# Graph-COM/HEPT

Hardware: AMD Instinct MI355X
Metric: attention-fwd points/sec (higher is better)
Workload: dtype bf16

## Files before the change

### hept_amd/csrc/block_attn.hip

```cpp
#include "common.h"
#include "p2p_dev.h"

namespace {

#ifndef HEPT_ATTN_STORE
#define HEPT_ATTN_STORE 1
#endif
__device__ __forceinline__ void store16_rows(unsigned int* dst, const u32x4& v) {
#if HEPT_ATTN_STORE == 1
    __builtin_nontemporal_store(v, reinterpret_cast<u32x4*>(dst));
#else
    *reinterpret_cast<u32x4*>(dst) = v;
#endif
}

#ifndef HEPT_RAGGED16_WAVES
#define HEPT_RAGGED16_WAVES 7
#endif
constexpr int attn_waves(int nkt, bool bf16, bool p16, bool full, bool diff = false) {
    if (diff) return full ? 3 : 2;
    return bf16 ? ((nkt == 3 && !p16 && full) ? 6 : (full ? 8 : HEPT_RAGGED16_WAVES)) : (full ? 6 : 4);
}
template <int NKT, bool BF16, bool P16, bool F16QK, bool FULL, bool DIFF = false>
__global__ __launch_bounds__(64 * NKT) __attribute__((amdgpu_waves_per_eu(attn_waves(NKT, BF16, P16, FULL, DIFF), attn_waves(NKT, BF16, P16, FULL, DIFF))))
void block_attn_kernel(const char* __restrict__ qhat,
                                                              const char* __restrict__ kvhat,
                                                              const int* __restrict__ qpos,
                                                              const int* __restrict__ kpos,
                                                              float* __restrict__ part, int N, int H, int D, int B,
                                                              int nb, HeadRange hr, PushArgs pa) {
    if (pa.push_wgs > 0 && (int)blockIdx.x < pa.push_wgs) {
        reduce_push_body<P16>(pa, (int)blockIdx.x);
        return;
    }
    constexpr int NT = 64 * NKT;
    constexpr int KEYS = 32 * NKT;
    constexpr int ESZ = BF16 ? 2 : 4;
    constexpr int QROW = 32 * ESZ;
    constexpr int KVROW = 2 * QROW;
    constexpr int CH = QROW / 16;
    constexpr int CPR = 2 * CH;

    extern __shared__ __attribute__((aligned(16))) char smem[];
    char* k_s = smem;
    char* v_s = smem + KEYS * QROW;
    float* kn_s = reinterpret_cast<float*>(smem + 2 * KEYS * QROW);
    int* qidx_s = reinterpret_cast<int*>(smem + 2 * KEYS * QROW + KEYS * 4);

    const int tid = threadIdx.x, lane = tid & 63, w = tid >> 6, hh = lane >> 5, li = lane & 31;
    const int bid = (int)blockIdx.x - pa.push_wgs;
    const int h = hr.h0 + bid % hr.hg;
    const int rest = bid / hr.hg;
    const int b = hr.tl > 0 ? rest / hr.tl : rest % nb, t = hr.tl > 0 ? rest % hr.tl : rest / nb;
    const size_t seg = ((size_t)t * H + h) * N + (size_t)b * B;
    const int* __restrict__ kp = kpos + seg;
    const int* __restrict__ qp = qpos + seg;
    const char* __restrict__ qbase = qhat + (size_t)h * N * QROW;
    const char* __restrict__ kvbase = kvhat + (size_t)h * N * KVROW;

    const int qi = w * 32 + li;
    const bool qvalid = FULL || qi < B;
    const int qsrc = qp[qvalid ? qi : 0];
    if (hh == 0) qidx_s[qi] = qvalid ? qsrc : -1;
    const char* qrow = qbase + (size_t)qsrc * QROW;
    float qn = *reinterpret_cast<const float*>(qrow + QROW - 4);
    u32x4 qraw[BF16 ? 2 : 4];
#pragma unroll
    for (int s = 0; s < (BF16 ? 2 : 4); ++s)
        qraw[s] = *reinterpret_cast<const u32x4*>(qrow + (BF16 ? (s * 32 + hh * 16) : (hh * 64 + s * 16)));
    if (hh == 1) qraw[BF16 ? 1 : 3][3] = 0u;
    if constexpr (DIFF) {
        static_assert(!BF16, "the difference form runs on f32 rows");
        float part = 0.f;
#pragma unroll
        for (int s2 = 0; s2 < 4; ++s2)
#pragma unroll
            for (int j = 0; j < 4; ++j) {
                const bool feat = 16 * hh + 4 * s2 + j < D;
                const float qv = __uint_as_float(qraw[s2][j]);
                part = feat ? fmaf(qv, qv, part) : part;
                if (!feat) qraw[s2][j] = 0u;
            }
        qn = -0.5f * (part + __shfl_xor(part, 32));
    }

#pragma unroll
    for (int it = 0; it < CPR / 2; ++it) {
        const int ci = it * NT + tid;
        const int key = ci / CPR, c = ci % CPR;
        u32x4 val = {0u, 0u, 0u, 0u};
        if (FULL || key < B) {
            const int src = kp[key];
            val = *reinterpret_cast<const u32x4*>(kvbase + (size_t)src * KVROW + c * 16);
        }
        if (c < CH) {
            if (c == CH - 1) {
                kn_s[key] = __uint_as_float(val[3]);
                val[3] = 0u;
            }
            const int sw = BF16 ? ((key >> 2) & 3) : ((key >> 1) & 7);
            *reinterpret_cast<u32x4*>(k_s + key * QROW + ((c ^ sw) * 16)) = val;
        } else {
            *reinterpret_cast<u32x4*>(v_s + key * QROW + (c - CH) * 16) = val;
        }
    }
    __syncthreads();
    if constexpr (DIFF) {
        if (tid < KEYS) {
            const int sw = (tid >> 1) & 7;
            float acc = 0.f;
            for (int col = 0; col < D; ++col) {
                const float kv2 = *reinterpret_cast<const float*>(k_s + tid * QROW + (((col >> 2) ^ sw) * 16) + (col & 3) * 4);
                acc = fmaf(kv2, kv2, acc);
            }
            kn_s[tid] = -0.5f * acc;
        }
        __syncthreads();
    }

    f32x16 z;
#pragma unroll
    for (int r = 0; r < 16; ++r) z[r] = 0.f;

#pragma unroll
    for (int kt = 0; kt < NKT; ++kt) {
        if (!FULL && kt * 32 >= B) break;
        const int key = kt * 32 + li;
        f32x16 x;
#pragma unroll
        for (int r = 0; r < 16; ++r) x[r] = qn + kn_s[kt * 32 + hept_acc_row(r, hh)];

        if constexpr (BF16) {
#pragma unroll
            for (int s = 0; s < 2; ++s) {
                const int c = 2 * s + hh;
                const u32x4 kraw =
                    *reinterpret_cast<const u32x4*>(k_s + key * QROW + ((c ^ ((key >> 2) & 3)) * 16));
                if constexpr (F16QK)
                    x = __builtin_amdgcn_mfma_f32_32x32x16_f16(__builtin_bit_cast(f16x8, kraw),
                                                               __builtin_bit_cast(f16x8, qraw[s]), x, 0, 0, 0);
                else
                    x = __builtin_amdgcn_mfma_f32_32x32x16_bf16(__builtin_bit_cast(bf16x8, kraw),
                                                                __builtin_bit_cast(bf16x8, qraw[s]), x, 0, 0, 0);
            }
        } else {
            float kf[16];
#pragma unroll
            for (int c = 0; c < 4; ++c) {
                const f32x4 kk = *reinterpret_cast<const f32x4*>(
                    k_s + key * QROW + (((4 * hh + c) ^ ((key >> 1) & 7)) * 16));
                kf[4 * c] = kk[0]; kf[4 * c + 1] = kk[1]; kf[4 * c + 2] = kk[2]; kf[4 * c + 3] = kk[3];
            }
#pragma unroll
            for (int s = 0; s < 16; ++s)
                x = __builtin_amdgcn_mfma_f32_32x32x2f32(kf[s], __uint_as_float(qraw[s >> 2][s & 3]), x, 0, 0, 0);
            if constexpr (DIFF) {
                float dsq[16];
#pragma unroll
                for (int r = 0; r < 16; ++r) dsq[r] = 0.f;
                for (int col = D; col < 30; ++col) {
                    const float qc = *reinterpret_cast<const float*>(qrow + col * 4);
#pragma unroll
                    for (int r = 0; r < 16; ++r) {
                        const int kr = kt * 32 + hept_acc_row(r, hh);
                        const float kc = *reinterpret_cast<const float*>(
                            k_s + kr * QROW + (((col >> 2) ^ ((kr >> 1) & 7)) * 16) + (col & 3) * 4);
                        const float dlt = qc - kc;
                        dsq[r] = fmaf(dlt, dlt, dsq[r]);
                    }
                }
#pragma unroll
                for (int r = 0; r < 16; ++r) x[r] = fmaf(-0.5f, dsq[r], x[r]);
            }
        }

        float pr[16];
        exp_clamped(x, pr);
        if (!FULL && (kt + 1) * 32 > B) {
#pragma unroll
            for (int r = 0; r < 16; ++r)
                if (kt * 32 + hept_acc_row(r, hh) >= B) pr[r] = 0.f;
        }

        if constexpr (BF16) {
            const int g = lane >> 4, l16 = lane & 15;
            const int vrow = kt * 32 + 4 * hh + (l16 >> 2);
            const int vcol = 32 * (g & 1) + 8 * (l16 & 3);
#pragma unroll
            for (int s = 0; s < 2; ++s) {
                u32x4 pw;
#pragma unroll
                for (int j = 0; j < 4; ++j) pw[j] = hept_pack_bf16(pr[8 * s + 2 * j], pr[8 * s + 2 * j + 1]);
                const s16x4 v0 = __builtin_amdgcn_ds_read_tr16_b64_v4i16(
                    (lds_s16x4_ptr)(v_s + (vrow + 16 * s) * QROW + vcol));
                const s16x4 v1 = __builtin_amdgcn_ds_read_tr16_b64_v4i16(
                    (lds_s16x4_ptr)(v_s + (vrow + 16 * s + 8) * QROW + vcol));
                typedef __attribute__((ext_vector_type(8))) short s16x8;
                const s16x8 vv = {v0[0], v0[1], v0[2], v0[3], v1[0], v1[1], v1[2], v1[3]};
                z = __builtin_amdgcn_mfma_f32_32x32x16_bf16(__builtin_bit_cast(bf16x8, pw),
                                                            __builtin_bit_cast(bf16x8, vv), z, 0, 0, 0);
            }
        } else {
#pragma unroll
            for (int r = 0; r < 16; ++r) {
                const float vv =
                    *reinterpret_cast<const float*>(v_s + (kt * 32 + hept_acc_row(r, hh)) * QROW + li * 4);
                z = __builtin_amdgcn_mfma_f32_32x32x2f32(pr[r], vv, z, 0, 0, 0);
            }
        }
    }

    if constexpr (P16) {
        __syncthreads();
        float* tile = reinterpret_cast<float*>(smem) + w * 32 * 32;
        {
            float* wr = tile + (4 * hh) * 32 + li;
#pragma unroll
            for (int r = 0; r < 16; ++r) wr[((r & 3) + 8 * (r >> 2)) * 32] = z[r];
        }
        unsigned int* __restrict__ pt =
            reinterpret_cast<unsigned int*>(part) + (size_t)t * hr.tstride_rows * 16 + (size_t)(h - hr.hsub) * 16;
#pragma unroll
        for (int j = 0; j < 2; ++j) {
            const int row = (lane >> 2) + 16 * j, pc = lane & 3;
            const int q2 = w * 32 + row;
            const f32x4 f0 = *reinterpret_cast<const f32x4*>(tile + row * 32 + pc * 8);
            const f32x4 f1 = *reinterpret_cast<const f32x4*>(tile + row * 32 + pc * 8 + 4);
            u32x4 v = {hept_pack_bf16(f0[0], f0[1]), hept_pack_bf16(f0[2], f0[3]), hept_pack_bf16(f1[0], f1[1]),
                       hept_pack_bf16(f1[2], f1[3])};
            if (pc == 3) v = u32x4{__float_as_uint(f0[0] + 1e-20f), 0u, 0u, 0u};
            if (FULL || q2 < B) {
                const int dst = qidx_s[q2];
                if (pa.direct) {
                    bool remote;
                    char* rowp = direct_row(pa, dst, h - hr.h0, 64, remote) + pc * 16;
                    if (remote) store16_system(rowp, v);
                    else *reinterpret_cast<u32x4*>(rowp) = v;
                } else {
                    store16_rows(pt + (size_t)dst * hr.hout * 16 + pc * 4, v);
                }
            }
        }
    } else {
        float* __restrict__ pt = part + (size_t)t * hr.tstride_rows * 32 + (size_t)(h - hr.hsub) * 32 + li;
#pragma unroll
        for (int r = 0; r < 16; ++r) {
            const int q2 = w * 32 + hept_acc_row(r, hh);
            if (FULL || q2 < B) {
                const int dst = qidx_s[q2];
                float val = z[r];
                if (li == D) val += 1e-20f;
                if (pa.direct) {
                    bool remote;
                    char* rowp = direct_row(pa, dst, h - hr.h0, 128, remote) + li * 4;
                    if (remote) store4_system(rowp, __float_as_uint(val));
                    else *reinterpret_cast<float*>(rowp) = val;
                } else {
                    pt[(size_t)dst * hr.hout * 32] = val;
                }
            }
        }
    }
    if (pa.direct) {
        drain_remote_stores();
        if (pa.counter) signal_when_all_done(pa.counter, pa.peers, pa.world, pa.flag_idx, pa.epoch, gridDim.x - pa.push_wgs);
    }
}

#ifndef HEPT_SPLIT_CK8
#define HEPT_SPLIT_CK8 128
#endif
constexpr int split_ck(int nkt) { return nkt == 8 ? HEPT_SPLIT_CK8 : (nkt >= 2 ? 64 : 32); }
#ifndef HEPT_SPLIT_PP
#define HEPT_SPLIT_PP 2
#endif
template <int NKT, bool FULL, int VP, bool DIFF = false>
__global__ __launch_bounds__(64 * NKT) void block_attn_split_kernel(const float* __restrict__ qhat,
                                                                    const float* __restrict__ kvhat,
                                                                    const int* __restrict__ qpos,
                                                                    const int* __restrict__ kpos,
                                                                    float* __restrict__ part, int N, int H, int D,
                                                                    int B, int nb, HeadRange hr, PushArgs pa) {
    if (pa.push_wgs > 0 && (int)blockIdx.x < pa.push_wgs) {
        reduce_push_body<false>(pa, (int)blockIdx.x);
        return;
    }
    constexpr int NT = 64 * NKT;
    constexpr int KEYS = 32 * NKT;
    constexpr int PROW = 64;
    constexpr int CK = split_ck(NKT);
    constexpr int NCH = (KEYS + CK - 1) / CK;
    constexpr int IPT = (CK * 8 + NT - 1) / NT;
    extern __shared__ __attribute__((aligned(16))) char smem[];
    char* k_s = smem;
    char* v_s = smem + 3 * CK * PROW;
    float* kc_s = reinterpret_cast<float*>(smem + (3 + VP) * CK * PROW);

    const int tid = threadIdx.x, lane = tid & 63, w = tid >> 6, hh = lane >> 5, li = lane & 31;
    const int bid = (int)blockIdx.x - pa.push_wgs;
    const int h = hr.h0 + bid % hr.hg;
    const int rest = bid / hr.hg;
    const int b = hr.tl > 0 ? rest / hr.tl : rest % nb, t = hr.tl > 0 ? rest % hr.tl : rest / nb;
    const size_t seg = ((size_t)t * H + h) * N + (size_t)b * B;
    const int* __restrict__ kp = kpos + seg;
    const int* __restrict__ qp = qpos + seg;
    const float* __restrict__ qbase = qhat + (size_t)h * N * 32;
    const float* __restrict__ kvbase = kvhat + (size_t)h * N * 64;

    float pre[IPT][8];
    auto fetch = [&](int ch) {
#pragma unroll
        for (int it = 0; it < IPT; ++it) {
            const int ci = it * NT + tid;
            const int key = ch * CK + (ci >> 3), c = ci & 7;
#pragma unroll
            for (int j = 0; j < 8; ++j) pre[it][j] = 0.f;
            if (ci < CK * 8 && key < (FULL ? KEYS : B)) {
                const int ks = kp[key];
                if (c >= 4 && hr.vsrc) {
                    const int col = 8 * (c - 4);
                    const float* src = hr.vsrc + ((size_t)ks * H + h) * D + col;
                    const bool real = ks < hr.raw_size;
                    if (real && col < D) {
                        const f32x4 a0 = *reinterpret_cast<const f32x4*>(src);
                        pre[it][0] = a0[0]; pre[it][1] = a0[1]; pre[it][2] = a0[2]; pre[it][3] = a0[3];
                    }
                    if (real && col + 4 < D) {
                        const f32x4 a1 = *reinterpret_cast<const f32x4*>(src + 4);
                        pre[it][4] = a1[0]; pre[it][5] = a1[1]; pre[it][6] = a1[2]; pre[it][7] = a1[3];
                    }
                    if (col == D) pre[it][0] = 1.f;
                    if (col + 4 == D) pre[it][4] = 1.f;
                } else {
                    const float* src = kvbase + (size_t)ks * 64 + c * 8;
                    const f32x4 a0 = *reinterpret_cast<const f32x4*>(src);
                    const f32x4 a1 = *reinterpret_cast<const f32x4*>(src + 4);
                    pre[it][0] = a0[0]; pre[it][1] = a0[1]; pre[it][2] = a0[2]; pre[it][3] = a0[3];
                    pre[it][4] = a1[0]; pre[it][5] = a1[1]; pre[it][6] = a1[2]; pre[it][7] = a1[3];
                    if (c == 3) pre[it][6] = 1.f;
                }
            }
        }
    };
    auto stage = [&]() {
#pragma unroll
        for (int it = 0; it < IPT; ++it) {
            const int ci = it * NT + tid;
            if (ci >= CK * 8) break;
            const int row = ci >> 3, c = ci & 7;
            u32x4 ph, pm, pl;
            if constexpr (DIFF) {
                float sq = 0.f;
                if (c < 3) {
#pragma unroll
                    for (int j = 0; j < 8; ++j) sq = fmaf(pre[it][j], pre[it][j], sq);
                }
                const int sqi = __builtin_bit_cast(int, sq);
                const float s1 = __builtin_bit_cast(float, __builtin_amdgcn_update_dpp(0, sqi, 0x111, 0xF, 0xF, true));
                const float s2 = __builtin_bit_cast(float, __builtin_amdgcn_update_dpp(0, sqi, 0x112, 0xF, 0xF, true));
                const float s3 = __builtin_bit_cast(float, __builtin_amdgcn_update_dpp(0, sqi, 0x113, 0xF, 0xF, true));
                if (c == 3) {
                    *reinterpret_cast<f32x4*>(kc_s + row * 8) = f32x4{pre[it][0], pre[it][1], pre[it][2], pre[it][3]};
                    *reinterpret_cast<f32x4*>(kc_s + row * 8 + 4) = f32x4{pre[it][4], pre[it][5], 0.f, 0.f};
#pragma unroll
                    for (int j = 0; j < 6; ++j) pre[it][j] = 0.f;
                    pre[it][7] = -0.5f * ((s3 + s2) + s1);
                }
            }
            if (c < 4) {
                split3_bf16(pre[it], ph, pm, pl);
                const int off = row * PROW + ((c ^ ((row >> 2) & 3)) * 16);
                *reinterpret_cast<u32x4*>(k_s + off) = ph;
                *reinterpret_cast<u32x4*>(k_s + CK * PROW + off) = pm;
                *reinterpret_cast<u32x4*>(k_s + 2 * CK * PROW + off) = pl;
            } else {
                if constexpr (VP == 3) split3_bf16(pre[it], ph, pm, pl);
                else split2_bf16(pre[it], ph, pm);
                const int off = row * PROW + (c - 4) * 16;
                *reinterpret_cast<u32x4*>(v_s + off) = ph;
                *reinterpret_cast<u32x4*>(v_s + CK * PROW + off) = pm;
                if constexpr (VP == 3) *reinterpret_cast<u32x4*>(v_s + 2 * CK * PROW + off) = pl;
            }
        }
    };
    fetch(0);

    const int qi = w * 32 + li;
    const bool qvalid = FULL || qi < B;
    const int qsrc = qp[qvalid ? qi : 0];
    const float* qrow = qbase + (size_t)qsrc * 32;
    u32x4 qh[2], qm[2], ql[2];
    float qc[DIFF ? 6 : 1];
    {
        float av[2][8];
#pragma unroll
        for (int s = 0; s < 2; ++s) {
            const f32x4 a0 = *reinterpret_cast<const f32x4*>(qrow + 16 * s + 8 * hh);
            const f32x4 a1 = *reinterpret_cast<const f32x4*>(qrow + 16 * s + 8 * hh + 4);
            av[s][0] = a0[0]; av[s][1] = a0[1]; av[s][2] = a0[2]; av[s][3] = a0[3];
            av[s][4] = a1[0]; av[s][5] = a1[1]; av[s][6] = a1[2]; av[s][7] = a1[3];
        }
        if constexpr (DIFF) {
            float fn = 0.f;
#pragma unroll
            for (int j = 0; j < 8; ++j) fn = fmaf(av[0][j], av[0][j], fn);
            if (hh == 0) {
#pragma unroll
                for (int j = 0; j < 8; ++j) fn = fmaf(av[1][j], av[1][j], fn);
            }
            fn += __shfl_xor(fn, 32);
#pragma unroll
            for (int c = 0; c < 6; ++c) qc[c] = __shfl(av[1][c], li + 32);
            if (hh == 1) {
#pragma unroll
                for (int j = 0; j < 6; ++j) av[1][j] = 0.f;
                av[1][6] = -0.5f * fn;
                av[1][7] = 1.f;
            }
        } else if (hh == 1) {
            av[1][6] = av[1][7];
            av[1][7] = 1.f;
        }
#pragma unroll
        for (int s = 0; s < 2; ++s) split3_bf16(av[s], qh[s], qm[s], ql[s]);
    }

    f32x16 z;
#pragma unroll
    for (int r = 0; r < 16; ++r) z[r] = 0.f;
    const int krow[2] = {li * PROW + ((hh ^ ((li >> 2) & 3)) * 16), li * PROW + (((2 + hh) ^ ((li >> 2) & 3)) * 16)};
    const int vlane = (4 * hh + ((lane & 15) >> 2)) * PROW + 32 * ((lane >> 4) & 1) + 8 * (lane & 3);

#pragma unroll
    for (int ch = 0; ch < NCH; ++ch) {
        if (!FULL && ch * CK >= B) break;
        if (ch > 0) __syncthreads();
        stage();
        if (ch + 1 < NCH) fetch(ch + 1);
        __syncthreads();
        constexpr int TPC = CK / 32, GRP = TPC < 2 ? TPC : 2;
#pragma unroll
        for (int g0 = 0; g0 < TPC; g0 += GRP) {
        f32x16 xs[GRP];
#pragma unroll
        for (int kg = 0; kg < GRP; ++kg) {
            const int kl = g0 + kg;
            const int kt = ch * TPC + kl;
            if (kt >= NKT) break;
            if (!FULL && kt * 32 >= B) break;
#pragma unroll
            for (int r = 0; r < 16; ++r) xs[kg][r] = 0.f;
#pragma unroll
            for (int s = 0; s < 2; ++s) {
                const int off = kl * 32 * PROW + krow[s];
                const u32x4 kh = *reinterpret_cast<const u32x4*>(k_s + off);
                const u32x4 km = *reinterpret_cast<const u32x4*>(k_s + CK * PROW + off);
                const u32x4 kl3 = *reinterpret_cast<const u32x4*>(k_s + 2 * CK * PROW + off);
                xs[kg] = mfma_bf16(kl3, qh[s], xs[kg]);
                xs[kg] = mfma_bf16(kh, ql[s], xs[kg]);
                xs[kg] = mfma_bf16(km, qm[s], xs[kg]);
                xs[kg] = mfma_bf16(km, qh[s], xs[kg]);
                xs[kg] = mfma_bf16(kh, qm[s], xs[kg]);
                xs[kg] = mfma_bf16(kh, qh[s], xs[kg]);
            }
        }
#pragma unroll
        for (int kg = 0; kg < GRP; ++kg) {
            const int kl = g0 + kg;
            const int kt = ch * TPC + kl;
            if (kt >= NKT) break;
            if (!FULL && kt * 32 >= B) break;
            f32x16 x = xs[kg];
            if constexpr (DIFF) {
#pragma unroll
                for (int r = 0; r < 16; ++r) {
                    const float* kc = kc_s + (kl * 32 + hept_acc_row(r, hh)) * 8;
                    const f32x4 k0 = *reinterpret_cast<const f32x4*>(kc), k1 = *reinterpret_cast<const f32x4*>(kc + 4);
                    float d0 = qc[0] - k0[0], d1 = qc[1] - k0[1], d2 = qc[2] - k0[2], d3 = qc[3] - k0[3];
                    float d4 = qc[4] - k1[0], d5 = qc[5] - k1[1];
                    float dsq = d0 * d0;
                    dsq = fmaf(d1, d1, dsq); dsq = fmaf(d2, d2, dsq); dsq = fmaf(d3, d3, dsq);
                    dsq = fmaf(d4, d4, dsq); dsq = fmaf(d5, d5, dsq);
                    x[r] = fmaf(-0.5f, dsq, x[r]);
                }
            }

            float pr[16];
            exp_clamped(x, pr);
            if (!FULL && (kt + 1) * 32 > B) {
#pragma unroll
                for (int r = 0; r < 16; ++r)
                    if (kt * 32 + hept_acc_row(r, hh) >= B) pr[r] = 0.f;
            }

#pragma unroll
            for (int s = 0; s < 2; ++s) {
                float pa[8];
#pragma unroll
                for (int j = 0; j < 8; ++j) pa[j] = pr[8 * s + j];
                constexpr int PP = HEPT_SPLIT_PP;
                u32x4 pp[3];
                if constexpr (PP == 3) split3_bf16(pa, pp[0], pp[1], pp[2]);
                else split2_bf16(pa, pp[0], pp[1]);
                typedef __attribute__((ext_vector_type(8))) short s16x8;
                u32x4 vpl[VP];
#pragma unroll
                for (int pl = 0; pl < VP; ++pl) {
                    const char* vb = v_s + pl * CK * PROW + (kl * 32 + 16 * s) * PROW + vlane;
                    const s16x4 v0 = __builtin_amdgcn_ds_read_tr16_b64_v4i16((lds_s16x4_ptr)(vb));
                    const s16x4 v1 = __builtin_amdgcn_ds_read_tr16_b64_v4i16((lds_s16x4_ptr)(vb + 8 * PROW));
                    const s16x8 vv = {v0[0], v0[1], v0[2], v0[3], v1[0], v1[1], v1[2], v1[3]};
                    vpl[pl] = __builtin_bit_cast(u32x4, vv);
                }
#pragma unroll
                for (int ord = 2; ord >= 0; --ord)
#pragma unroll
                    for (int i = PP - 1; i >= 0; --i) {
                        const int j = ord - i;
                        if (j >= 0 && j < VP) z = mfma_bf16(pp[i], vpl[j], z);
                    }
            }
        }
        }
    }

    __syncthreads();
    float* tile = reinterpret_cast<float*>(smem) + w * 32 * 32;
    {
        float* wr = tile + (4 * hh) * 32 + li;
#pragma unroll
        for (int r = 0; r < 16; ++r) wr[((r & 3) + 8 * (r >> 2)) * 32] = z[r];
    }
    float* __restrict__ pt = part + (size_t)t * hr.tstride_rows * 32 + (size_t)(h - hr.hsub) * 32;
#pragma unroll
    for (int j = 0; j < 4; ++j) {
        const int row = (lane >> 3) + 8 * j, pc = lane & 7;
        const int q2 = w * 32 + row;
        const int dst = __shfl(qsrc, row);
        f32x4 f = *reinterpret_cast<const f32x4*>(tile + row * 32 + pc * 4);
#pragma unroll
        for (int e = 0; e < 4; ++e)
            if (pc * 4 + e == D) f[e] += 1e-20f;
        if (FULL || q2 < B) {
            if (pa.direct) {
                bool remote;
                char* rowp = direct_row(pa, dst, h - hr.h0, 128, remote) + pc * 16;
                if (remote) store16_system(rowp, __builtin_bit_cast(u32x4, f));
                else *reinterpret_cast<f32x4*>(rowp) = f;
            } else {
                *reinterpret_cast<f32x4*>(pt + (size_t)dst * hr.hout * 32 + pc * 4) = f;
            }
        }
    }
    if (pa.direct) {
        drain_remote_stores();
        if (pa.counter) signal_when_all_done(pa.counter, pa.peers, pa.world, pa.flag_idx, pa.epoch, gridDim.x - pa.push_wgs);
    }
}

template <bool FULL, int VP, bool DIFF = false>
int launch_attn_split(int nkt, dim3 grid, hipStream_t st, const float* qhat, const float* kvhat, const int* qpos,
                      const int* kpos, float* part, int N, int H, int D, int B, int nb, HeadRange hr, PushArgs pa) {
#define HEPT_SPLIT_CASE(K)                                                                                       \
    case K: {                                                                                                    \
                          \
        constexpr size_t lds0 = (size_t)(3 + VP) * split_ck(K) * 64 + (DIFF ? (size_t)split_ck(K) * 32 : 0);        \
        constexpr size_t lds = lds0 > (size_t)K * 4096 ? lds0 : (size_t)K * 4096;                                \
        if (lds > 65536) {                                                                                       \
            static LdsRaised raised;                                                                             \
            if (hept_raise_lds(raised, reinterpret_cast<const void*>(&block_attn_split_kernel<K, FULL, VP, DIFF>), lds)) \
                return HEPT_ERR_LAUNCH;                                                                          \
        }                                                                                                        \
        hipLaunchKernelGGL((block_attn_split_kernel<K, FULL, VP, DIFF>), grid, dim3(64 * K), lds, st, qhat, kvhat, qpos, \
                           kpos, part, N, H, D, B, nb, hr, pa);                                                        \
        break;                                                                                                   \
    }
    switch (nkt) {
        HEPT_SPLIT_CASE(1)
        HEPT_SPLIT_CASE(2)
        HEPT_SPLIT_CASE(3)
        HEPT_SPLIT_CASE(4)
        HEPT_SPLIT_CASE(5)
        HEPT_SPLIT_CASE(6)
        HEPT_SPLIT_CASE(7)
        HEPT_SPLIT_CASE(8)
        default:
            return HEPT_ERR_SHAPE;
    }
#undef HEPT_SPLIT_CASE
    return hept_launch_status();
}

template <bool BF16, bool P16, bool F16QK, bool FULL, bool DIFF = false>
int launch_attn_full(int nkt, dim3 grid, hipStream_t st, const char* qhat, const char* kvhat, const int* qpos,
                const int* kpos, float* part, int N, int H, int D, int B, int nb, HeadRange hr, PushArgs pa) {
#define HEPT_ATTN_CASE(K)                                                                                    \
    case K: {                                                                                                \
        constexpr size_t lds = (size_t)2 * 32 * K * 32 * (BF16 ? 2 : 4) + 32 * K * 8;                        \
        if (lds > 65536) {                                                                                   \
            static LdsRaised raised;                                                                         \
            if (hept_raise_lds(raised, reinterpret_cast<const void*>(&block_attn_kernel<K, BF16, P16, F16QK, FULL, DIFF>), lds)) \
                return HEPT_ERR_LAUNCH;                                                                      \
        }                                                                                                    \
        hipLaunchKernelGGL((block_attn_kernel<K, BF16, P16, F16QK, FULL, DIFF>), grid, dim3(64 * K), lds, st, qhat, kvhat, qpos, \
                           kpos, part, N, H, D, B, nb, hr, pa);                                                    \
        break;                                                                                               \
    }
    switch (nkt) {
        HEPT_ATTN_CASE(1)
        HEPT_ATTN_CASE(2)
        HEPT_ATTN_CASE(3)
        HEPT_ATTN_CASE(4)
        HEPT_ATTN_CASE(5)
        HEPT_ATTN_CASE(6)
        HEPT_ATTN_CASE(7)
        HEPT_ATTN_CASE(8)
        default:
            return HEPT_ERR_SHAPE;
    }
#undef HEPT_ATTN_CASE
    return hept_launch_status();
}

template <bool BF16, bool P16, bool F16QK, bool DIFF = false>
int launch_attn(int nkt, dim3 grid, hipStream_t st, const char* qhat, const char* kvhat, const int* qpos,
                const int* kpos, float* part, int N, int H, int D, int B, int nb, HeadRange hr, PushArgs pa) {
    if (B == 32 * nkt)
        return launch_attn_full<BF16, P16, F16QK, true, DIFF>(nkt, grid, st, qhat, kvhat, qpos, kpos, part, N, H, D, B, nb, hr, pa);
    return launch_attn_full<BF16, P16, F16QK, false, DIFF>(nkt, grid, st, qhat, kvhat, qpos, kpos, part, N, H, D, B, nb, hr, pa);
}

}

namespace {
int block_attn_impl(const void* qhat, const void* kvhat, const int32_t* qpos, const int32_t* kpos, int N, int H, int D,
                    int Tl, int B, int precision, const HeadRange& hr_in, float* part, void* stream,
                    const PushArgs* push = nullptr, VSrc vs = VSrc{}) {
    HeadRange hr = hr_in;
    hr.vsrc = nullptr;
    hr.raw_size = N;
    static const bool table_major = [] { const char* e = getenv("HEPT_ATTN_TABLE_MAJOR"); return e && *e && *e != '0'; }();
    hr.tl = table_major ? 0 : Tl;
    if (vs.v) {
        if (precision != HEPT_PREC_F32 || D % 4 != 0 || (reinterpret_cast<uintptr_t>(vs.v) & 15)) return HEPT_ERR_ARG;
        hr.vsrc = vs.v;
        hr.raw_size = vs.raw_size;
    }
    if (!qhat || !kvhat || !qpos || !kpos || (!part && !(push && push->direct))) return HEPT_ERR_ARG;
    if (N < 1 || H < 1 || Tl < 1 || B < 1 || B > HEPT_MAX_BLOCK || N % B != 0 || D < 1 || D > 28)
        return HEPT_ERR_SHAPE;
    if (hr.h0 < 0 || hr.hg < 1 || hr.h0 + hr.hg > H || hr.hout < 1 || hr.hsub < 0 || hr.hsub > hr.h0 ||
        hr.h0 + hr.hg - hr.hsub > hr.hout)
        return HEPT_ERR_SHAPE;

    const int nb = N / B, nkt = (B + 31) / 32;
    PushArgs pa{};
    if (push) {
        pa = *push;
        if (pa.direct ? (pa.push_wgs != 0 || Tl != 1 || pa.h0 != hr.h0 || pa.hg != hr.hg) : pa.push_wgs < 1)
            return HEPT_ERR_ARG;
    }
    const dim3 grid((unsigned)((size_t)Tl * nb * hr.hg + pa.push_wgs));
    hipStream_t st = (hipStream_t)stream;
    const char* qh = (const char*)qhat;
    const char* kv = (const char*)kvhat;
    if (precision == HEPT_PREC_BF16 && D == 24)
        return launch_attn<true, true, false>(nkt, grid, st, qh, kv, qpos, kpos, part, N, H, D, B, nb, hr, pa);
    if (precision == HEPT_PREC_BF16)
        return launch_attn<true, false, false>(nkt, grid, st, qh, kv, qpos, kpos, part, N, H, D, B, nb, hr, pa);
    if (precision == HEPT_PREC_MIXED16 && D == 24)
        return launch_attn<true, true, true>(nkt, grid, st, qh, kv, qpos, kpos, part, N, H, D, B, nb, hr, pa);
    if (precision == HEPT_PREC_MIXED16)
        return launch_attn<true, false, true>(nkt, grid, st, qh, kv, qpos, kpos, part, N, H, D, B, nb, hr, pa);
    if (precision == HEPT_PREC_F32) {
        const float* qf = (const float*)qhat;
        const float* kf = (const float*)kvhat;
        if (B == 32 * nkt) return launch_attn_split<true, 3>(nkt, grid, st, qf, kf, qpos, kpos, part, N, H, D, B, nb, hr, pa);
        return launch_attn_split<false, 3>(nkt, grid, st, qf, kf, qpos, kpos, part, N, H, D, B, nb, hr, pa);
    }
    if (precision == HEPT_PREC_F32_MFMA)
        return launch_attn<false, false, false>(nkt, grid, st, qh, kv, qpos, kpos, part, N, H, D, B, nb, hr, pa);
    if (precision == HEPT_PREC_F32_DIFF) {
        const char* e = getenv("HEPT_DIFF_MFMA");
        const bool mfma = e && *e && *e != '0';
        if (D == 24 && !mfma) {
            const float* qf = (const float*)qhat;
            const float* kf = (const float*)kvhat;
            if (B == 32 * nkt) return launch_attn_split<true, 3, true>(nkt, grid, st, qf, kf, qpos, kpos, part, N, H, D, B, nb, hr, pa);
            return launch_attn_split<false, 3, true>(nkt, grid, st, qf, kf, qpos, kpos, part, N, H, D, B, nb, hr, pa);
        }
        return launch_attn<false, false, false, true>(nkt, grid, st, qh, kv, qpos, kpos, part, N, H, D, B, nb, hr, pa);
    }
    return HEPT_ERR_SHAPE;
}
}

int hept_block_attn_heads_push(const void* qhat, const void* kvhat, const int32_t* qpos, const int32_t* kpos, int N,
                               int H, int D, int Tl, int B, int precision, int h0, int hg, int hout, int hsub,
                               int n_rows_out, float* part, const PushArgs* push, void* stream, VSrc vs) {
    if (n_rows_out < N) return HEPT_ERR_SHAPE;
    const HeadRange hr{h0, hg, hout, hsub, (long long)n_rows_out * hout, nullptr, 0, 0};
    return block_attn_impl(qhat, kvhat, qpos, kpos, N, H, D, Tl, B, precision, hr, part, stream, push, vs);
}

extern "C" int hept_block_attn(const void* qhat, const void* kvhat, const int32_t* qpos, const int32_t* kpos, int N,
                               int H, int D, int Tl, int B, int precision, float* part, void* stream) {
    const HeadRange all{0, H, H, 0, (long long)N * H, nullptr, 0, 0};
    return block_attn_impl(qhat, kvhat, qpos, kpos, N, H, D, Tl, B, precision, all, part, stream);
}

extern "C" int hept_block_attn_heads(const void* qhat, const void* kvhat, const int32_t* qpos, const int32_t* kpos,
                                     int N, int H, int D, int Tl, int B, int precision, int h0, int hg, int hout,
                                     int hsub, int n_rows_out, float* part, void* stream) {
    if (n_rows_out < N) return HEPT_ERR_SHAPE;
    const HeadRange hr{h0, hg, hout, hsub, (long long)n_rows_out * hout, nullptr, 0, 0};
    return block_attn_impl(qhat, kvhat, qpos, kpos, N, H, D, Tl, B, precision, hr, part, stream);
}
```

Measured before the change: 372.8 million.

## Prefetch key positions two chunks ahead and make K/V fetch branch-free

```diff
diff --git a/hept_amd/csrc/block_attn.hip b/hept_amd/csrc/block_attn.hip
--- a/hept_amd/csrc/block_attn.hip
+++ b/hept_amd/csrc/block_attn.hip
@@ -307,48 +307,72 @@
     const float* __restrict__ qbase = qhat + (size_t)h * N * 32;
     const float* __restrict__ kvbase = kvhat + (size_t)h * N * 64;
 
+    const int c = tid & 7;
+    const bool vs = c >= 4 && hr.vsrc;
+    auto item_ok = [&](int ch, int it) {
+        const int ci = it * NT + tid;
+        return (IPT * NT == CK * 8 || ci < CK * 8) && ((FULL && NCH * CK == KEYS) || ch * CK + (ci >> 3) < (FULL ? KEYS : B));
+    };
+    const int qi = w * 32 + li;
+    const bool qvalid = FULL || qi < B;
+    const int qsrc = qp[qvalid ? qi : 0];
+    int kpr[2][IPT];
+    auto positions = [&](int ch) {
+#pragma unroll
+        for (int it = 0; it < IPT; ++it) kpr[ch & 1][it] = kp[item_ok(ch, it) ? ch * CK + ((it * NT + tid) >> 3) : 0];
+    };
+    positions(0);
+    if (NCH > 1) positions(1);
     float pre[IPT][8];
     auto fetch = [&](int ch) {
 #pragma unroll
         for (int it = 0; it < IPT; ++it) {
-            const int ci = it * NT + tid;
-            const int key = ch * CK + (ci >> 3), c = ci & 7;
-#pragma unroll
-            for (int j = 0; j < 8; ++j) pre[it][j] = 0.f;
-            if (ci < CK * 8 && key < (FULL ? KEYS : B)) {
-                const int ks = kp[key];
-                if (c >= 4 && hr.vsrc) {
-                    const int col = 8 * (c - 4);
-                    const float* src = hr.vsrc + ((size_t)ks * H + h) * D + col;
-                    const bool real = ks < hr.raw_size;
-                    if (real && col < D) {
-                        const f32x4 a0 = *reinterpret_cast<const f32x4*>(src);
-                        pre[it][0] = a0[0]; pre[it][1] = a0[1]; pre[it][2] = a0[2]; pre[it][3] = a0[3];
-                    }
-                    if (real && col + 4 < D) {
-                        const f32x4 a1 = *reinterpret_cast<const f32x4*>(src + 4);
-                        pre[it][4] = a1[0]; pre[it][5] = a1[1]; pre[it][6] = a1[2]; pre[it][7] = a1[3];
-                    }
-                    if (col == D) pre[it][0] = 1.f;
-                    if (col + 4 == D) pre[it][4] = 1.f;
-                } else {
-                    const float* src = kvbase + (size_t)ks * 64 + c * 8;
-                    const f32x4 a0 = *reinterpret_cast<const f32x4*>(src);
-                    const f32x4 a1 = *reinterpret_cast<const f32x4*>(src + 4);
-                    pre[it][0] = a0[0]; pre[it][1] = a0[1]; pre[it][2] = a0[2]; pre[it][3] = a0[3];
-                    pre[it][4] = a1[0]; pre[it][5] = a1[1]; pre[it][6] = a1[2]; pre[it][7] = a1[3];
-                    if (c == 3) pre[it][6] = 1.f;
-                }
-            }
+            if (IPT * NT != CK * 8 && it * NT + tid >= CK * 8) break;
+            const int ks = kpr[ch & 1][it];
+            const float* s0 = kvbase + (size_t)ks * 64 + c * 8;
+            const float* s1 = s0 + 4;
+            if (vs) {
+                const int col = 8 * (c - 4);
+                const float* src = hr.vsrc + ((size_t)ks * H + h) * D + col;
+                const bool real = ks < hr.raw_size;
+                if (real && col < D) s0 = src;
+                if (real && col + 4 < D) s1 = src + 4;
+            }
+            const f32x4 a0 = *reinterpret_cast<const f32x4*>(s0);
+            const f32x4 a1 = *reinterpret_cast<const f32x4*>(s1);
+            pre[it][0] = a0[0]; pre[it][1] = a0[1]; pre[it][2] = a0[2]; pre[it][3] = a0[3];
+            pre[it][4] = a1[0]; pre[it][5] = a1[1]; pre[it][6] = a1[2]; pre[it][7] = a1[3];
         }
     };
-    auto stage = [&]() {
+    auto fixup = [&](int ch, int it) {
+        const bool ok = item_ok(ch, it);
+        if (vs) {
+            const int col = 8 * (c - 4);
+            const bool real = kpr[ch & 1][it] < hr.raw_size;
+            const bool k0 = ok && real && col < D, k1 = ok && real && col + 4 < D;
+#pragma unroll
+            for (int j = 0; j < 4; ++j) {
+                pre[it][j] = k0 ? pre[it][j] : 0.f;
+                pre[it][4 + j] = k1 ? pre[it][4 + j] : 0.f;
+            }
+            if (ok && col == D) pre[it][0] = 1.f;
+            if (ok && col + 4 == D) pre[it][4] = 1.f;
+        } else {
+            if (!ok) {
+#pragma unroll
+                for (int j = 0; j < 8; ++j) pre[it][j] = 0.f;
+            }
+            if (ok && c == 3) pre[it][6] = 1.f;
+        }
+    };
+    auto stage = [&](int ch) {
 #pragma unroll
         for (int it = 0; it < IPT; ++it) {
             const int ci = it * NT + tid;
             if (ci >= CK * 8) break;
-            const int row = ci >> 3, c = ci & 7;
+            const int row = ci >> 3;
             u32x4 ph, pm, pl;
+            fixup(ch, it);
             if constexpr (DIFF) {
                 float sq = 0.f;
                 if (c < 3) {
@@ -385,9 +409,6 @@
     };
     fetch(0);
 
-    const int qi = w * 32 + li;
-    const bool qvalid = FULL || qi < B;
-    const int qsrc = qp[qvalid ? qi : 0];
     const float* qrow = qbase + (size_t)qsrc * 32;
     u32x4 qh[2], qm[2], ql[2];
     float qc[DIFF ? 6 : 1];
@@ -435,8 +456,9 @@
     for (int ch = 0; ch < NCH; ++ch) {
         if (!FULL && ch * CK >= B) break;
         if (ch > 0) __syncthreads();
-        stage();
+        stage(ch);
         if (ch + 1 < NCH) fetch(ch + 1);
+        if (ch + 2 < NCH) positions(ch + 2);
         __syncthreads();
         constexpr int TPC = CK / 32, GRP = TPC < 2 ? TPC : 2;
 #pragma unroll
```

New measurement: 370.9 million. Within noise of the previous version (-0.5%).
